# sefffal/Octofitter.jl

Hardware: AMD Instinct MI355X
Metric: epoch-likelihood evals/sec (fwd+grad), 1e4 epochs x 1e4 walkers (higher is better)
Workload: dtype f64; 1 GPU; config3: 1 planet, 10000 RA/Dec epochs x 10000 walkers in total (10000 walkers split over 1 GPUs: 10000 walkers/GPU), fwd+reverse-grad, inputs and outputs resident in HBM (PCIe-inclusive rate: value_pcie_inclusive); walkers_per_gpu=10000, walkers_total=10000, rows=10000, parallelism=walkers sharded x1, dataset replicated, no data-path collective

## Files before the change

### octofitter.jl_amd/csrc/octo_api.hip

```cpp
#define OCTO_API_TU 1
#include "octo_host.h"
#include "octo_tile.h"

using namespace octo;

namespace octo {

std::atomic<uint64_t> g_dataset_serial{1};

int fail(octo_ctx* ctx, int code, const std::string& msg) {
    if (ctx) ctx->err = msg;
    return code;
}

int busy(octo_ctx* ctx, const char* what) {
    if (ctx->pending.active) return fail(ctx, OCTO_EINVAL, std::string(what) + ": an octo_eval_begin of this context has not been ended");
    return OCTO_OK;
}


DevConsts dev_consts(const octo_consts& c) {
    DevConsts d;
    d.k_yr = c.kepler_year_to_julian_day; d.yd = c.year2day_julian; d.au2m = c.au2m; d.sec2yr = c.sec2year_julian;
    d.mas_per_au_per_plx = c.rad2as / c.pc2au;
// ... 219 lines not shown
    if (rounds != 1 || ctx->env_rounds > 0 || n_rows < 32 * WPB * 8) return key0;
    const int64_t t_max = std::max<int64_t>(1, n_rows / (32 * WPB));
    int64_t best_t = key0;
    double best_cost = 1e300;
    for (int wps = 1; wps <= blocks_per_cu; ++wps) {
        int64_t t = std::min<int64_t>((int64_t)wps * n_cus / cols, t_max);
        if (t < 1) continue;
        const double chunk = std::ceil((double)n_rows / (double)(t * WPB));
        const double n = std::ceil((double)(cols * t) / (double)n_cus);
        static const double g[8] = {1.59, 1.59, 1.13, 1.045, 1.03, 1.015, 1.005, 1.0};
        const double cost = n * g[(int)std::min(n, 7.0)] * (chunk + 2.7) + 0.34 * (double)t;
        if (cost < best_cost) { best_cost = cost; best_t = t; }
    }
    if (wide && ctx->env_wide >= 0) {
        const double n4 = std::ceil((double)(cols * best_t) / (double)n_cus);
        *wide = (n4 <= (double)blocks8_per_cu && n_rows >= (int64_t)best_t * 8 * 32) || (ctx->env_wide > 0 && n4 <= (double)blocks8_per_cu);
    }
    return best_t;
}

bool small_eligible(const octo_ctx* ctx, const octo_dataset* ds, int64_t W, bool model) {
    if (ctx->opt_invariant) return false;
    if (ds->n_planets > MAXP_T) return false;
    const int limit = (model && ds->n_planets == 1) ? std::max(ctx->small_w, ctx->small_w_model) : ctx->small_w;
    if (!(W * ds->n_planets <= limit && W <= SMALL_W)) return false;
    if (ds->kind_mask & KM_MARG)
        for (int o = 0; o < ds->n_obs; ++o)
            if (ds->h_obs[o].kind == OCTO_RV_ABS_MARG && ds->h_obs[o].n > SMALL_MARG_ROWS) return false;
    return true;
}

constexpr int TILE_PROBE_EVERY = 64;
constexpr double TILE_COLD_ROW_US = 27.0 * 2.15e-3;
constexpr double TILE_LAUNCH_US = 6.5;

static int tile_settle(octo_ctx* ctx, const octo_dataset* ds) {
    HIPCHK(ctx, hipEventSynchronize(ctx->ev_tile));
    double d = 0.0;
    for (int k = 0; k < ctx->tile_pending_segs; ++k) d += (double)ctx->h_tile_stats[2 * k] - (double)ctx->h_tile_stats[2 * k + 1];
    ctx->tile_last_saving_us = d * (double)ds->tile_rows * TILE_COLD_ROW_US / (4.0 * (double)ctx->n_cus);
    ctx->tile_on = ctx->tile_last_saving_us > 1.3 * TILE_LAUNCH_US;
    ctx->tile_pending = false;
    return OCTO_OK;
}

int tile_prepare(octo_ctx* ctx, const octo_dataset* ds, EvalArgs& a, hipStream_t st) {
    a.perm = nullptr;
    const int kp = ds->n_planets - 1;
    if (!a.warm || ctx->tile_mode == 0 || a.W < ctx->tile_min_w || !(ds->tile_dm_ref > 0.0f) || ds->n_planets > 2 ||
        ds->planets[kp].orbit_kind == OCTO_ORBIT_THIELE_INNES)
        return OCTO_OK;
    bool probe = false, sort_now = ctx->tile_mode == 1;
    if (ctx->tile_mode == 2 && ds->n_planets > 1) return OCTO_OK;
    if (ctx->tile_mode == 2) {
        if (ctx->tile_ds != ds->serial || ctx->tile_W != a.W) {
            ctx->tile_ds = ds->serial; ctx->tile_W = a.W; ctx->tile_seq = 0; ctx->tile_on = false; ctx->tile_pending = false;
        }
        if (ctx->tile_pending) { int rcd = tile_settle(ctx, ds); if (rcd) return rcd; }
        probe = (ctx->tile_seq % TILE_PROBE_EVERY) == 0;
        ctx->tile_seq += 1;
        sort_now = ctx->tile_on;
    }
    if (!sort_now && !probe) return OCTO_OK;
    const int n_seg = (int)((a.W + TILE_SEG - 1) / TILE_SEG);
    int rc = grow(ctx, ctx->d_perm, ctx->cap_perm, a.W);
    if (rc) return rc;
    if (2 * (int64_t)n_seg > ctx->cap_tile_stats) {
        if (ctx->h_tile_stats) ctx->retired_host.push_back((void*)ctx->h_tile_stats);
        ctx->h_tile_stats = nullptr; ctx->cap_tile_stats = 0;
        const int64_t n = 2 * (int64_t)n_seg + 64;
        HIPCHK(ctx, hipHostMalloc((void**)&ctx->h_tile_stats, sizeof(float) * (size_t)n, hipHostMallocMapped | hipHostMallocPortable | hipHostMallocCoherent));
        ctx->cap_tile_stats = n;
    }
    if (!ctx->ev_tile) HIPCHK(ctx, hipEventCreateWithFlags(&ctx->ev_tile, hipEventDisableTiming));
    TileArgs ta;
    ta.elems = a.elems; ta.ld = a.ld; ta.W = a.W; ta.perm = ctx->d_perm; ta.stats = probe ? ctx->h_tile_stats : nullptr;
    ta.dm_ref = ds->tile_dm_ref; ta.inv_k_yr = (float)(1.0 / ctx->consts.kepler_year_to_julian_day);
    ta.planet = kp; ta.pad = 0;
    hipLaunchKernelGGL(k_tile_sort, dim3((unsigned)n_seg), dim3(TILE_TPB), 0, st, ta);
    if (probe) {
        HIPCHK(ctx, hipEventRecord(ctx->ev_tile, st));
        ctx->tile_pending = true; ctx->tile_pending_segs = n_seg; ctx->tile_probes += 1;
        if (ctx->tile_seq == 1) {
            int rcd = tile_settle(ctx, ds);
            if (rcd) return rcd;
            sort_now = ctx->tile_on;
        }
    }
    if (sort_now) { ctx->tile_sorted_launches += 1; a.perm = ctx->d_perm; }
    return OCTO_OK;
}

int drain_timing(octo_ctx* ctx) {
    for (size_t k = 0; k < ctx->ev_used; ++k) {
        float ms = 0.f;
        HIPCHK(ctx, hipEventSynchronize(ctx->ev_pool[k].second));
        HIPCHK(ctx, hipEventElapsedTime(&ms, ctx->ev_pool[k].first, ctx->ev_pool[k].second));
        ctx->t_ms += ms;
        ctx->t_n += 1;
        if (ctx->t_samples.size() < (1u << 20)) ctx->t_samples.push_back(ms);
    }
    ctx->ev_used = 0;
    return OCTO_OK;
}

}

extern "C" {

int32_t octo_consts_default(octo_consts* out) {
    if (!out) return OCTO_EINVAL;
    out->kepler_year_to_julian_day = 365.2568983840419;
    out->year2day_julian = 365.25;
    out->au2m = 1.495978707e11;
    out->sec2year_julian = 3.168808781402895e-8;
// ... 676 lines not shown
    if (sorted_launches) *sorted_launches = ctx->tile_sorted_launches;
    if (probes) *probes = ctx->tile_probes;
    if (on) *on = ctx->tile_on ? 1 : 0;
    if (last_saving_us) *last_saving_us = ctx->tile_last_saving_us;
    return OCTO_OK;
}

int32_t octo_debug_kepler_warm(octo_ctx* ctx, const double* MA, const double* dM, const double* e, int64_t n, double* sinE_out, double* cosE_out,
                               double* used_warm_out) {
    if (!ctx || !MA || !dM || !e || !sinE_out || !cosE_out || !used_warm_out || n < 0) return fail(ctx, OCTO_EINVAL, "octo_debug_kepler_warm: null argument");
    { int rcb = busy(ctx, "octo_debug_kepler_warm"); if (rcb) return rcb; }
    if (n == 0) return OCTO_OK;
    HIPCHK(ctx, hipSetDevice(ctx->device));
    int rc = grow(ctx, ctx->d_in, ctx->cap_in, 3 * n);
    if (rc) return rc;
    rc = grow(ctx, ctx->d_out, ctx->cap_out, 3 * n);
    if (rc) return rc;
    hipStream_t st;
    { int rcs = use_stream(ctx, OCTO_STREAM_CTX, &st); if (rcs) return rcs; }
    HIPCHK(ctx, hipMemcpyAsync(ctx->d_in, MA, sizeof(double) * n, hipMemcpyHostToDevice, st));
    HIPCHK(ctx, hipMemcpyAsync(ctx->d_in + n, dM, sizeof(double) * n, hipMemcpyHostToDevice, st));
    HIPCHK(ctx, hipMemcpyAsync(ctx->d_in + 2 * n, e, sizeof(double) * n, hipMemcpyHostToDevice, st));
    hipLaunchKernelGGL(k_kepler_warm, dim3((unsigned)((n + 255) / 256)), dim3(256), sizeof(double) * 2 * SCT_N, st, ctx->d_in, ctx->d_in + n, ctx->d_in + 2 * n, n,
                       ctx->d_out, ctx->d_out + n, ctx->d_out + 2 * n, ctx->d_sctab);
    HIPCHK(ctx, hipGetLastError());
    HIPCHK(ctx, hipMemcpyAsync(sinE_out, ctx->d_out, sizeof(double) * n, hipMemcpyDeviceToHost, st));
    HIPCHK(ctx, hipMemcpyAsync(cosE_out, ctx->d_out + n, sizeof(double) * n, hipMemcpyDeviceToHost, st));
    HIPCHK(ctx, hipMemcpyAsync(used_warm_out, ctx->d_out + 2 * n, sizeof(double) * n, hipMemcpyDeviceToHost, st));
    HIPCHK(ctx, hipStreamSynchronize(st));
    free_retired(ctx);
    return OCTO_OK;
}

int32_t octo_kepler_solve(octo_ctx* ctx, const double* MA, const double* e, int64_t n, double* E_out, double* sinE_out,
                          double* cosE_out) {
    return kepler_solve_host(ctx, MA, e, n, E_out, sinE_out, cosE_out, false);
}

int32_t octo_kepler_solve_table(octo_ctx* ctx, const double* MA, const double* e, int64_t n, double* E_out, double* sinE_out,
                                double* cosE_out) {
    return kepler_solve_host(ctx, MA, e, n, E_out, sinE_out, cosE_out, true);
}

int32_t octo_timing_enable(octo_ctx* ctx, int32_t on) {
    if (!ctx) return OCTO_EINVAL;
    ctx->timing_every = on > 0 ? on : 0;
    ctx->timing_whole = on < 0;
    ctx->timing_seq = 0;
    return OCTO_OK;
}

int32_t octo_timing_read(octo_ctx* ctx, double* avg_ms, int64_t* n_launches, int32_t reset) {
    if (!ctx) return OCTO_EINVAL;
    HIPCHK(ctx, hipSetDevice(ctx->device));
    int rc = drain_timing(ctx);
    if (rc) return rc;
    if (avg_ms) *avg_ms = ctx->t_n > 0 ? ctx->t_ms / (double)ctx->t_n : 0.0;
    if (n_launches) *n_launches = ctx->t_n;
    if (reset) { ctx->t_ms = 0.0; ctx->t_n = 0; ctx->t_samples.clear(); }
    return OCTO_OK;
}

int32_t octo_timing_stats(octo_ctx* ctx, double* median_ms, double* min_ms, double* max_ms, int64_t* n_launches) {
    if (!ctx) return OCTO_EINVAL;
    HIPCHK(ctx, hipSetDevice(ctx->device));
    int rc = drain_timing(ctx);
// ... 504 lines not shown
```

### octofitter.jl_amd/csrc/octo_device.h

```cpp
#pragma once
#include <hip/hip_runtime.h>
#include <stdint.h>

namespace octo {

constexpr int WAVE = 64;
constexpr double PI = 3.141592653589793238462643383279502884;
constexpr double TWO_PI = 6.283185307179586476925286766559005768;
constexpr double PI2 = PI * PI;
constexpr double LOG2PI = 1.8378770664093454835606594728112;
constexpr double MK_K0 = 3.0 * PI2 / (PI2 - 6.0);
constexpr double MK_K1N = 8.0 * PI / (5.0 * (PI2 - 6.0));

enum : int {
    WC_INVP = 0,
    WC_TP,
    WC_E,
    WC_BETA,
    WC_EOB,
    WC_CB, WC_CG, WC_CA, WC_CF,
    WC_K,
    WC_COSW, WC_SINW,
    WC_MU,
    WC_A,
// ... 235 lines not shown
    const double u = s.dt * pc.invP;
    const double frac = u - rint(u);
    const float E1f = markley_starter_f32(frac, pc);
    const double E1 = (double)E1f;
    double s1, c1;
    if constexpr (TAB) sincos_table(E1f, tab, s1, c1);
    else sincos_halfangle(E1, s1, c1);
    const double f0 = fma(-pc.e, s1, fma(-frac, TWO_PI, E1));
    kepler_correct<INV_NR>(s, pc, E1, s1, c1, f0);
    return s;
}

template <int INV_NR>
__device__ __forceinline__ KSol kepler_warm_step(double t, const PC& pc, KWarm& st, double dm) {
    static_assert(INV_NR >= 0, "the warm start needs 1/(1 − e cos E) of every row");
    KSol s;
    s.dt = t - pc.tp;
    const double dM = dm * pc.invP;
    const double x = dM * st.invD;
    const double z = x * st.invD;
    const double dE = fma(-((pc.he * st.sE) * z), x, x);
    const double u = dE * dE;
    const double sr = dE * fma(u, fma(u, fma(u, OCTO_KT[22], OCTO_KT[17]), OCTO_KT[18]), 1.0);
    const double cm1 = u * fma(u, fma(u, fma(u, OCTO_KT[23], OCTO_KT[19]), OCTO_KT[20]), -0.5);
    const double ds = fma(st.sE, cm1, st.cE * sr);
    const double s1 = st.sE + ds;
    const double c1 = fma(st.cE, cm1, fma(-st.sE, sr, st.cE));
    const double f0 = fma(-pc.e, ds, dE - dM);
    kepler_correct<INV_NR, true>(s, pc, 0.0, s1, c1, f0);
    st.sE = s.sE; st.cE = s.cE; st.invD = s.invD;
    return s;
}

#ifndef OCTO_WARM_TRI
#define OCTO_WARM_TRI 1
#endif
template <int INV_NR, bool TRI = (OCTO_WARM_TRI != 0)>
__device__ __forceinline__ KSol kepler_solve_warm(double t, const PC& pc, const SinCosTab& tab, KWarm& st, double thr, double dm, bool row_ok = true) {
    static_assert(INV_NR >= 0, "the warm start needs 1/(1 − e cos E) of every row");
    KSol s;
    s.dt = t - pc.tp;
    double E1 = 0.0, s1, c1, f0;
    const bool warm_row = row_ok && __builtin_amdgcn_ballot_w64(st.invD >= thr) == 0;
    if constexpr (TRI) {
    {
        const double dM = dm * pc.invP;
        const double x = dM * st.invD;
        const double z = x * st.invD;
        const double dE = fma(-((pc.he * st.sE) * z), x, x);
        const double u = dE * dE;
        const double sr = dE * fma(u, fma(u, fma(u, OCTO_KT[22], OCTO_KT[17]), OCTO_KT[18]), 1.0);
        const double cm1 = u * fma(u, fma(u, fma(u, OCTO_KT[23], OCTO_KT[19]), OCTO_KT[20]), -0.5);
        const double ds = fma(st.sE, cm1, st.cE * sr);
        s1 = st.sE + ds;
        c1 = fma(st.cE, cm1, fma(-st.sE, sr, st.cE));
        f0 = fma(-pc.e, ds, dE - dM);
        kepler_correct<INV_NR, true>(s, pc, E1, s1, c1, f0);
    }
#ifndef OCTO_WARM_NOREDO
    if (__builtin_expect(!warm_row, 0)) {
        const double uo = s.dt * pc.invP;
        const double frac = uo - rint(uo);
        const float E1f = markley_starter_f32(frac, pc);
        E1 = (double)E1f;
        sincos_table(E1f, tab, s1, c1);
        f0 = fma(-pc.e, s1, fma(-frac, TWO_PI, E1));
// ... 33 lines not shown
```

### octofitter.jl_amd/csrc/octo_host.h

```cpp
#pragma once
#include <hip/hip_runtime.h>

#include <algorithm>
#include <atomic>
#include <cmath>
#include <cstdio>
#include <cstdlib>
#include <cstring>
#include <map>
#include <mutex>
#include <new>
#include <string>
#include <vector>

#include "octo_kernels.h"
#include "octo_model.h"
#include "octo_hgca.h"
#include "octo_small.h"
#include "octofitter_hip.h"

namespace octo {

struct TaskTable {
    uint64_t ds_serial = 0;
// ... 55 lines not shown
    double* d_marg = nullptr;
    double* d_extra = nullptr;
    int64_t cap_extra = 0;
    double* d_sctab = nullptr;
    int32_t* d_counters = nullptr;
    uint64_t* h_flags = nullptr;
    uint64_t flag_seq = 0;
    bool flag_request = false, flag_armed = false;
    SmallInline inl = {};
    int64_t stage_ws_in = 0, stage_ws_out = 0;
    struct ModelTail { const double *Jc = nullptr, *gtp = nullptr, *glp = nullptr, *lpp = nullptr; const octo_source *esrc = nullptr, *nsrc = nullptr; double *lp = nullptr, *grad = nullptr; int64_t ld = 0, ldo = 0; int32_t D = 0, n_nu = 0; };
    bool mt_applied = false;
    struct Pending {
        bool active = false, staged = false, walker_major = false;
        int64_t W = 0, ld = 0, ldd = 0, ws_out = 0, o_ge = 0, o_gn = 0;
        int n_el_out = 0, n_nu_out = 0;
        double *ll = nullptr, *g_elems = nullptr, *g_nuis = nullptr;
    } pending;
    void* comm = nullptr;
    int comm_rank = 0, comm_world = 1;
    int small_w_model = 768;
    int small_w = OCTO_SMALL_BATCH_DEFAULT;
    int64_t env_small_blocks = 0, env_small_min_span = 0, env_stage_bytes = 0, env_chunk = 0, env_rounds = 0, env_rv_cost = 0, env_kind_all = 0, env_mainp_tpb = 0;
    int env_warm = 1;
    int opt_warm = 1;
    int opt_invariant = 0;
    int tile_mode = 2;
    int64_t tile_min_w = 2048;
    int32_t* d_perm = nullptr; int64_t cap_perm = 0;
    float* h_tile_stats = nullptr; int64_t cap_tile_stats = 0;
    hipEvent_t ev_tile = nullptr;
    bool tile_on = false, tile_pending = false;
    int tile_pending_segs = 0;
    int64_t tile_seq = 0, tile_W = 0, tile_sorted_launches = 0, tile_probes = 0;
    uint64_t tile_ds = 0;
    double tile_last_saving_us = 0.0;
    int env_no_fin_fused = 0;
    int env_wide = 0;
    int flag_w = 128;
    int mapped_w = 128;
    double *d_in = nullptr, *d_out = nullptr;
    int64_t cap_in = 0, cap_out = 0;
    double *h_in = nullptr, *h_out = nullptr;
    int64_t cap_hin = 0, cap_hout = 0;
    std::vector<void*> retired_host;
    std::vector<void*> retired;
    std::vector<octo::TaskTable> tables;
    std::map<uint32_t, int> occupancy;
    std::map<const void*, size_t> lds_raised;
    int timing_every = 0;
    bool timing_whole = false;
    int64_t timing_seq = 0;
    std::vector<std::pair<hipEvent_t, hipEvent_t>> ev_pool;
    size_t ev_used = 0;
    double t_ms = 0.0;
    int64_t t_n = 0;
    std::vector<float> t_samples;
};


namespace octo {

int fail(octo_ctx* ctx, int code, const std::string& msg);

#define HIPCHK(ctx, call)                                                                          \
    do {                                                                                           \
// ... 57 lines not shown
```

### octofitter.jl_amd/csrc/octo_kernels.h

```cpp
#pragma once
#include <type_traits>

#include "octo_device.h"
#include "octofitter_hip.h"

namespace octo {

constexpr int MAXP = OCTO_MAX_PLANETS;
constexpr int MAXP_T = OCTO_MAX_PLANETS_ALL_KINDS;
constexpr int ROW_STRIDE = 8;
constexpr int WPB = 4;
#ifndef OCTO_FIN_G
#define OCTO_FIN_G 16
#endif
#ifndef OCTO_FIN_UNROLL
#define OCTO_FIN_UNROLL 4
#endif
constexpr int FIN_G = OCTO_FIN_G;
constexpr int fin_nwr(int n_planets) { return n_planets == 2 ? 3 : (n_planets == 3 ? 2 : 1); }
#ifndef OCTO_FIN_CH
#define OCTO_FIN_CH 6
#endif
#ifndef OCTO_FIN_FAST
#define OCTO_FIN_FAST true
// ... 288 lines not shown
    const KSol s = kepler_solve<2, TAB>(MA[i], pc, tab);
    const bool ok = (e >= 0.0) && (e < 1.0) && isfinite(MA[i]);
    E[i] = ok ? s.E : NAN;
    if (sE) sE[i] = ok ? s.sE : NAN;
    if (cE) cE[i] = ok ? s.cE : NAN;
}

static __global__ __launch_bounds__(256) void k_kepler_warm(const double* __restrict__ MA, const double* __restrict__ dMa, const double* __restrict__ ecc,
                                                            int64_t n, double* sE, double* cE, double* used, const double* __restrict__ sctab) {
    extern __shared__ __attribute__((aligned(16))) double lds[];
    const SinCosTab tab = make_sincos_tab(reinterpret_cast<const double2*>(lds));
    {
        const double2* __restrict__ g = reinterpret_cast<const double2*>(sctab);
        double2* t = reinterpret_cast<double2*>(lds);
        for (int i = threadIdx.x; i < SCT_N; i += blockDim.x) t[i] = g[i];
        __syncthreads();
    }
    const int64_t i0 = (int64_t)blockIdx.x * blockDim.x + threadIdx.x;
    const int64_t i = i0 < n ? i0 : n - 1;
    PC pc = {};
    const double e = ecc[i];
    pc.invP = 1.0 / TWO_PI; pc.tp = 0.0; pc.e = e; pc.beta = sqrt(1.0 - e * e); pc.eob = e / pc.beta;
    set_starter(pc, (float)e, (float)(1.0 - e), (float)(MK_K1N / (1.0 + e)));
    const KSol s0 = kepler_solve<2, true>(MA[i], pc, tab);
    KWarm st{s0.sE, s0.cE, s0.invD};
    const float dmx = fabsf((float)dMa[i]);
    double thr = (double)__builtin_amdgcn_exp2f(0.2f * (__builtin_amdgcn_logf((float)WARM_TOL) - 3.0f * __builtin_amdgcn_logf(dmx)));
    if (thr < WARM_MIN_THR) thr = 0.0;
    const bool warm = __builtin_amdgcn_ballot_w64(st.invD >= thr) == 0;
    const KSol s = kepler_solve_warm<2>(MA[i] + dMa[i], pc, tab, st, thr, dMa[i] * TWO_PI);
    if (i0 < n) { sE[i] = s.sE; cE[i] = s.cE; used[i] = warm ? 1.0 : 0.0; }
}

#endif

template <int P>
struct AstromCoef {
    double f[P];
    double jit, j2, ps, na, sn, cn;
    bool seppa, oneil;
    int planet, has_cor;
};

template <int P, bool GRAD, bool NUIS, int KM>
__device__ __forceinline__ AstromCoef<P> astrom_coef_vals(double jit, double ps, double na, int ob_kind, int ob_planet, int ob_has_cor, const PC (&pc)[P]) {
    using L = Layout<P, GRAD, NUIS, KM>;
    AstromCoef<P> c;
    if constexpr (P == 1) {
        c.f[0] = 1.0;
    } else {
        double a_this = 0.0;
#pragma unroll
        for (int p = 0; p < P; ++p) a_this = (p == ob_planet) ? pc[p].a : a_this;
#pragma unroll
        for (int p = 0; p < P; ++p) c.f[p] = (p == ob_planet) ? 1.0 : ((pc[p].a < a_this) ? pc[p].mu : 0.0);
    }
    c.jit = 0.0; c.j2 = 0.0; c.ps = 1.0; c.na = 0.0; c.sn = 0.0; c.cn = 1.0;
    if constexpr (NUIS) {
        c.jit = jit; c.ps = ps; c.na = na;
        sincos_reduced(c.na, c.sn, c.cn);
        c.j2 = c.jit * c.jit;
    }
    c.seppa = (KM & KM_SEPPA) && (ob_kind == OCTO_ASTROM_SEPPA || ob_kind == OCTO_ONEIL_SEPPA);
    c.oneil = L::HAS_ONEIL && (ob_kind == OCTO_ONEIL_RADEC || ob_kind == OCTO_ONEIL_SEPPA);
    c.planet = ob_planet; c.has_cor = ob_has_cor;
    return c;
}

template <int P, bool GRAD, bool NUIS, int KM>
__device__ __forceinline__ AstromCoef<P> astrom_coef(const double* __restrict__ nuis, int64_t ld, int ob_kind, int ob_planet, int ob_has_cor,
                                                     int obs_index, const PC (&pc)[P], int64_t wl) {
    double jit = 0.0, ps = 1.0, na = 0.0;
    if constexpr (NUIS) {
        const double* nu = nuis + (int64_t)obs_index * OCTO_N_NUIS * ld + wl;
        jit = nu[OCTO_NU_JITTER * ld]; ps = nu[OCTO_NU_PLATESCALE * ld]; na = nu[OCTO_NU_NORTHANGLE * ld];
    }
    return astrom_coef_vals<P, GRAD, NUIS, KM>(jit, ps, na, ob_kind, ob_planet, ob_has_cor, pc);
}

template <int P>
struct WarmState { KWarm st[P]; double thr[P]; uint32_t key_hi; bool row_ok; };

template <int P, bool GRAD, bool NUIS, int KM, bool TAB, int WARM = 0, bool WCHECK = true, int WLAST = 0>
__device__ __forceinline__ void astrom_row(AccArr<P, GRAD, NUIS, KM>& acc, LogProd& lp, const PC (&pc)[P],
                                           const AstromCoef<P>& co, double t, double y1, double y2, double c3, double c4, double c5,
                                           const SinCosTab& tab, WarmState<P>* ws = nullptr, double dm = 0.0) {
    using L = Layout<P, GRAD, NUIS, KM>;
    constexpr bool DEFER = TAB;
    const double (&f)[P] = co.f;
    const double jit = co.jit, j2 = co.j2, ps = co.ps, na = co.na, sn = co.sn, cn = co.cn;
    const bool seppa = co.seppa, oneil = co.oneil;
    KSol s[P];
    double rap[P], dep[P];
    double ra_m, dec_m;
#pragma unroll
    for (int p = 0; p < P; ++p) {
        if constexpr (WARM != 0) s[p] = kepler_solve_warm<1, WARM == 1>(t, pc[p], tab, ws->st[p], ws->thr[p], dm, WCHECK ? ws->row_ok : true);
        else if constexpr (WLAST != 0) { if (p == P - 1) s[p] = kepler_warm_step<1>(t, pc[p], ws->st[p], dm); else s[p] = kepler_solve<1, TAB>(t, pc[p], tab); }
        else s[p] = kepler_solve<1, TAB>(t, pc[p], tab);
        if constexpr (WLAST == 2) {
            if (p == P - 1 && __builtin_expect(!ws->row_ok, 0)) {
                s[p] = kepler_solve<1, TAB>(t, pc[p], tab);
                ws->st[p].sE = s[p].sE; ws->st[p].cE = s[p].cE; ws->st[p].invD = s[p].invD;
            }
        }
        rap[p] = fma(pc[p].cB, s[p].cE, fma(pc[p].cGb, s[p].sE, -pc[p].cBe));
        dep[p] = fma(pc[p].cA, s[p].cE, fma(pc[p].cFb, s[p].sE, -pc[p].cAe));
    }
    if constexpr (L::HAS_ONEIL) {
        if (oneil) {
            double sE = 0.0, cE = 0.0, ee = 0.0, invD = 0.0, dtp = 0.0;
#pragma unroll
            for (int p = 0; p < P; ++p) {
                const bool me = (P == 1) || (p == co.planet);
                sE = me ? s[p].sE : sE; cE = me ? s[p].cE : cE; ee = me ? pc[p].e : ee; invD = me ? s[p].invD : invD; dtp = me ? s[p].dt : dtp;
            }
            double E = 0.0;
#pragma unroll
            for (int p = 0; p < P; ++p) E = ((P == 1) || (p == co.planet)) ? s[p].E : E;
            const double Mm = fma(-ee, sE, E);
            const double c2 = fma(ee, ee + cE, -2.0);
            const double tt = fma(3.0 * Mm, ee + cE, 2.0 * c2 * sE);
            acc[L::OFF_ONEIL] += fabs(tt);
            if constexpr (GRAD) {
                const double sg = tt < 0.0 ? -1.0 : 1.0;
                const double D = fma(-ee, cE, 1.0);
                const double tM = 3.0 * (ee + cE);
                const double tE = fma(-3.0 * Mm, sE, 2.0 * fma(c2, cE, -(ee * sE * sE))) + tM * D;
                const double te = fma(2.0 * sE, 2.0 * ee + cE, 3.0 * Mm) - tM * sE;
                const double Mb = sg * tE * invD;
// ... 327 lines not shown
template <int P, bool GRAD, bool NUIS, int KM>
constexpr size_t main_lds_bytes() { return sizeof(double) * (2 * SCT_N + Layout<P, GRAD, NUIS, KM>::NACC * WAVE); }
template <int P, bool GRAD, bool NUIS, int KM, int NWV = WPB>
constexpr size_t fused_lds_bytes() {
    const size_t b = main_lds_bytes<P, GRAD, NUIS, KM>(), c = sizeof(double) * (size_t)P * NPC * WAVE;
    const size_t d = NWV > WPB ? sizeof(double) * (size_t)(NWV - 1) * Layout<P, GRAD, NUIS, KM>::NACC * WAVE : 0;
    return b > c ? (b > d ? b : d) : (c > d ? c : d);
}

template <int P, bool GRAD, bool NUIS, int KM, int NWV = WPB>
constexpr unsigned main_min_waves() {
    if (P >= 4 && GRAD) return 2u;
    if (NWV == 2 * WPB && P == 1 && GRAD && !NUIS && (KM & ~KM_COR) == KM_RADEC) return 6u;
#ifdef OCTO_P2_WAVES
    if (P == 2 && GRAD && NUIS && !(KM & (KM_MARG | KM_ONEIL))) return (unsigned)OCTO_P2_WAVES;
#endif
    return 1u;
}

#ifndef OCTO_WARM
#define OCTO_WARM 1
#endif
#ifndef OCTO_WARM_PLAIN
#define OCTO_WARM_PLAIN 0
#endif
template <int P, bool GRAD, bool NUIS, int KM, bool FUSED>
constexpr bool main_warm_plain() {
    return OCTO_WARM && FUSED && P == 1 && !(KM & KM_ONEIL) && NUIS && ((KM & KM_SEPPA) || ((KM & KM_RV) && OCTO_WARM_PLAIN));
}
template <int P, bool GRAD, bool NUIS, int KM, bool FUSED>
constexpr bool main_warm() {
    return OCTO_WARM && FUSED && P == 1 && !(KM & KM_ONEIL);
}

#ifndef OCTO_WARM_LAST3
#define OCTO_WARM_LAST3 1
#endif
template <int P, bool GRAD, bool NUIS, int KM, bool FUSED>
constexpr bool main_warm_last() {
    return OCTO_WARM && FUSED && (P == 2 || (P == 3 && OCTO_WARM_LAST3 && !(KM & KM_SEPPA))) && !(KM & (KM_ONEIL | KM_MARG));
}

template <int P>
__device__ __forceinline__ float warm_last_init(WarmState<P>& ws, const PC& pc, const DevObs& ob, bool enabled) {
    float bound = 0.0f;
#pragma unroll
    for (int k = WARM_LADDER - 1; k >= 0; --k) {
        const float d = enabled ? ob.dm_ladder[k] : 0.0f;
        const bool veto = fabsf(d * (float)pc.invP) > WARM_DM_VETO;
        if (d > 0.0f && __builtin_amdgcn_ballot_w64(veto) == 0) bound = d;
    }
    ws.key_hi = (uint32_t)__builtin_amdgcn_readfirstlane(__double2hiint((double)bound));
    const float dmx = fabsf(bound * (1.0f + 0x1p-18f) * (float)pc.invP);
    const float th = __builtin_amdgcn_exp2f(0.2f * (__builtin_amdgcn_logf((float)WARM_TOL) - 3.0f * __builtin_amdgcn_logf(dmx)));
    ws.thr[P - 1] = (double)th;
    ws.st[P - 1].sE = 0.0; ws.st[P - 1].cE = 1.0; ws.st[P - 1].invD = __builtin_huge_val();
    return bound;
}

template <int P>
__device__ __forceinline__ float warm_init(WarmState<P>& ws, const PC (&pc)[P], const DevObs& ob, bool enabled) {
    float bound = 0.0f;
#pragma unroll
    for (int k = WARM_LADDER - 1; k >= 0; --k) {
        const float d = enabled ? ob.dm_ladder[k] : 0.0f;
        bool veto = false;
// ... 101 lines not shown
            double v[NWC];
            setup_assemble(v, elv[p], a.orbit_kind[p], raw[0 * WAVE], raw[1 * WAVE], raw[2 * WAVE], raw[3 * WAVE], raw[4 * WAVE], raw[5 * WAVE], q);
            pc[p].invP = v[WC_INVP]; pc[p].tp = v[WC_TP]; pc[p].e = v[WC_E]; pc[p].beta = v[WC_BETA]; pc[p].eob = v[WC_EOB];
            pc[p].cB = v[WC_CB]; pc[p].cG = v[WC_CG]; pc[p].cA = v[WC_CA]; pc[p].cF = v[WC_CF]; pc[p].K = v[WC_K]; pc[p].cw = v[WC_COSW];
            pc[p].sw = v[WC_SINW]; pc[p].mu = v[WC_MU]; pc[p].a = v[WC_A]; pc[p].cGb = v[WC_CGB]; pc[p].cFb = v[WC_CFB]; pc[p].cBe = v[WC_CBE];
            pc[p].cAe = v[WC_CAE];
            const float2 fa = *reinterpret_cast<const float2*>(&v[WC_F32A]);
            const float2 fb = *reinterpret_cast<const float2*>(&v[WC_F32B]);
            set_starter(pc[p], fa.x, fa.y, fb.x);
        }
        __syncthreads();
        {
            double2* t = reinterpret_cast<double2*>(lds);
#pragma unroll
            for (int k = 0; k < TPT; ++k) { const int i = (int)threadIdx.x + k * WAVE * NWV; if (i < SCT_N) t[i] = make_double2(trs[k], trc[k]); }
        }
    }

    double acc[L::NACC];
#pragma unroll
    for (int k = 0; k < L::NACC; ++k) acc[k] = 0.0;
    LogProd lp;
    __syncthreads();

    const bool is_astrom = ob.kind == OCTO_ASTROM_RADEC || ob.kind == OCTO_ASTROM_SEPPA || ob.kind == OCTO_ONEIL_RADEC ||
                           ob.kind == OCTO_ONEIL_SEPPA;

    if (L::HAS_ASTROM && (!L::HAS_RV || is_astrom)) {
        const AstromCoef<P> co = astrom_coef<P, GRAD, NUIS, KM>(a.nuis, a.ld, ob.kind, ob.planet, ob.has_cor, tk.obs, pc, wsrc);
        const crow_t rows = constant_rows((NUIS ? ob.raw : ob.pre) + (int64_t)row_first * ROW_STRIDE);
        auto body = [&](const RowRegs& r) {
            astrom_row<P, GRAD, NUIS, KM, true>(acc, lp, pc, co, row_get(r, 0), row_get(r, 1), row_get(r, 2), row_get(r, 3), row_get(r, 4), row_get(r, 5), tab);
        };
        bool warm_loop = false, warm_unchecked = false;
        WarmState<P> ws;
        if constexpr (main_warm<P, GRAD, NUIS, KM, FUSED>()) {
            const float bound = warm_init<P>(ws, pc, ob, a.warm != 0);
            warm_loop = bound > 0.0f;
            warm_unchecked = warm_loop && tk.key_max <= bound && tk.chunk <= WARM_RESTART;
        }
        bool warm_last = false;
        if constexpr (main_warm_last<P, GRAD, NUIS, KM, FUSED>()) {
            const float bound = warm_last_init<P>(ws, pc[P - 1], ob, a.warm != 0);
            warm_last = bound > 0.0f && n_rows > 0;
        }
        if (main_warm_last<P, GRAD, NUIS, KM, FUSED>() && warm_last) {
            if constexpr (main_warm_last<P, GRAD, NUIS, KM, FUSED>()) {
                auto lbody = [&](const RowRegs8& r) {
                    const uint64_t over = __builtin_amdgcn_ballot_w64(ws.st[P - 1].invD >= ws.thr[P - 1]);
                    ws.row_ok = ((uint32_t)warm_row_ok<P>(ws, r) & (uint32_t)(over == 0)) != 0;
                    astrom_row<P, GRAD, NUIS, KM, true, 0, true, 2>(acc, lp, pc, co, row_get(r, 0), row_get(r, 1), row_get(r, 2), row_get(r, 3), row_get(r, 4),
                                                                        row_get(r, 5), tab, &ws, row_get(r, 6));
                };
                RowRegs8 A = row_issue8(rows);
                for (int j = 0; j < n_rows; j += 2) {
                    RowRegs8 B = row_wait_issue(A, rows + (int64_t)(j + 1 < n_rows ? j + 1 : j) * ROW_STRIDE);
                    lbody(A);
                    if (__builtin_expect(j + 1 >= n_rows, 0)) { row_drain(B); break; }
                    A = row_wait_issue(B, rows + (int64_t)(j + 2 < n_rows ? j + 2 : j + 1) * ROW_STRIDE);
                    lbody(B);
                }
                row_drain(A);
            }
        } else if constexpr (!ROW_PREFETCH) {
            for (int j = 0; j < n_rows; ++j) {
                const crow_t rw = rows + (int64_t)j * ROW_STRIDE;
                astrom_row<P, GRAD, NUIS, KM, true>(acc, lp, pc, co, rw[0], rw[1], rw[2], rw[3], rw[4], rw[5], tab);
            }
        } else if (main_warm<P, GRAD, NUIS, KM, FUSED>() && warm_loop) {
            if constexpr (main_warm_plain<P, GRAD, NUIS, KM, FUSED>()) {
                for (int j = 0; j < n_rows; ++j) {
                    const crow_t rw = rows + (int64_t)j * ROW_STRIDE;
                    ws.row_ok = (uint32_t)__double2hiint(rw[7]) <= ws.key_hi;
                    astrom_row<P, GRAD, NUIS, KM, true, WMODE, true>(acc, lp, pc, co, rw[0], rw[1], rw[2], rw[3], rw[4], rw[5], tab, &ws, rw[6]);
                }
            } else if constexpr (main_warm<P, GRAD, NUIS, KM, FUSED>()) {
                auto wbody_t = [&](const RowRegs8& r, auto checked) {
                    if constexpr (decltype(checked)::value) ws.row_ok = warm_row_ok<P>(ws, r);
                    astrom_row<P, GRAD, NUIS, KM, true, WMODE, decltype(checked)::value>(acc, lp, pc, co, row_get(r, 0), row_get(r, 1), row_get(r, 2), row_get(r, 3),
                                                                                         row_get(r, 4), row_get(r, 5), tab, &ws, row_get(r, 6));
                };
                auto wloop = [&](auto checked) {
                    RowRegs8 A = row_issue8(rows);
                    for (int j = 0; j < n_rows; j += 2) {
                        RowRegs8 B = row_wait_issue(A, rows + (int64_t)(j + 1 < n_rows ? j + 1 : j) * ROW_STRIDE);
                        wbody_t(A, checked);
                        if (__builtin_expect(j + 1 >= n_rows, 0)) { row_drain(B); break; }
                        A = row_wait_issue(B, rows + (int64_t)(j + 2 < n_rows ? j + 2 : j + 1) * ROW_STRIDE);
                        wbody_t(B, checked);
                    }
                    row_drain(A);
                };
                if (n_rows > 0) {
                    if (warm_unchecked) wloop(std::false_type{});
                    else wloop(std::true_type{});
                }
            }
        } else if (n_rows > 0) {
            RowRegs A = row_issue(rows);
            for (int j = 0; j < n_rows; j += 2) {
                RowRegs B = row_wait_issue(A, rows + (int64_t)(j + 1 < n_rows ? j + 1 : j) * ROW_STRIDE);
                body(A);
                if (__builtin_expect(j + 1 >= n_rows, 0)) { row_drain(B); break; }
                A = row_wait_issue(B, rows + (int64_t)(j + 2 < n_rows ? j + 2 : j + 1) * ROW_STRIDE);
                body(B);
            }
            row_drain(A);
        }
        astrom_finish_sums<P, GRAD, NUIS, KM>(acc, co);
    }
    if (L::HAS_RV && !is_astrom) {
        const RvCoef<P> co = rv_coef<P, GRAD, NUIS, KM>(a.nuis, a.ld, a.marg, a.ldw, ob.kind, ob.planet, tk.obs, pc, wsrc);
        const crow_t rows = constant_rows((NUIS ? ob.raw : ob.pre) + (int64_t)row_first * ROW_STRIDE);
        auto body = [&](const RowRegs& r) {
            rv_row<P, GRAD, NUIS, KM, true>(acc, lp, pc, co, row_get(r, 0), row_get(r, 1), row_get(r, 2), NUIS ? row_get(r, 3) : 0.0, tab);
        };
        bool warm_loop = false, warm_unchecked = false;
        WarmState<P> ws;
        if constexpr (main_warm<P, GRAD, NUIS, KM, FUSED>()) {
            const float bound = warm_init<P>(ws, pc, ob, a.warm != 0);
            warm_loop = bound > 0.0f;
            warm_unchecked = warm_loop && tk.key_max <= bound && tk.chunk <= WARM_RESTART;
        }
        bool warm_last = false;
        if constexpr (main_warm_last<P, GRAD, NUIS, KM, FUSED>()) {
            const float bound = warm_last_init<P>(ws, pc[P - 1], ob, a.warm != 0);
            warm_last = bound > 0.0f && n_rows > 0;
// ... 857 lines not shown
```

### octofitter.jl_amd/csrc/octo_tile.h

```cpp
#pragma once
#include "octo_kernels.h"

namespace octo {

#ifndef OCTO_TILE_WPT
#define OCTO_TILE_WPT 1
#endif
constexpr int TILE_WPT = OCTO_TILE_WPT;
constexpr int TILE_TPB = 1024;
constexpr int TILE_SEG = TILE_TPB * TILE_WPT;
constexpr int TILE_K = 32;

struct TileArgs {
    const double* elems;
    int64_t ld, W;
    int32_t* perm;
    float* stats;
    float dm_ref;
    float inv_k_yr;
    int32_t planet;
    int32_t pad;
};

__device__ __forceinline__ float wave_excl_scan(float x, int lane, float& total) {
    float s = x;
#pragma unroll
    for (int d = 1; d < WAVE; d <<= 1) {
        const float y = __shfl_up(s, d, WAVE);
        if (lane >= d) s += y;
    }
    total = __shfl(s, WAVE - 1, WAVE);
    return s - x;
}

#ifdef OCTO_API_TU
static __global__ __launch_bounds__(TILE_TPB) void k_tile_sort(TileArgs a) {
    __shared__ __attribute__((aligned(16))) uint8_t cnt[TILE_K * TILE_TPB];
    __shared__ uint16_t goff[TILE_K * WAVE];
    __shared__ uint16_t bbase[TILE_K + 1];
    __shared__ float slq[TILE_SEG];
    __shared__ float red[2 * (TILE_TPB / WAVE)];
    const int t = threadIdx.x, lane = t & (WAVE - 1), wv = t >> 6;
    const int64_t seg0 = (int64_t)blockIdx.x * TILE_SEG;
    const int n_seg = (int)(a.W - seg0 < TILE_SEG ? a.W - seg0 : TILE_SEG);
    {
        uint4* z = reinterpret_cast<uint4*>(cnt);
        z[t] = make_uint4(0, 0, 0, 0); z[t + TILE_TPB] = make_uint4(0, 0, 0, 0);
#pragma unroll
        for (int i = 0; i < TILE_WPT; ++i) slq[TILE_WPT * t + i] = 0.0f;
    }
    int bk[TILE_WPT]; float lq[TILE_WPT];
#pragma unroll
    for (int i = 0; i < TILE_WPT; ++i) {
        const int k = TILE_WPT * t + i;
        bk[i] = -1; lq[i] = 0.0f;
        if (k >= n_seg) continue;
        const int64_t w = seg0 + k;
        const double* el = a.elems + (int64_t)a.planet * OCTO_N_EL * a.ld + w;
        const double sma = el[(int64_t)OCTO_EL_A * a.ld], ecc = el[(int64_t)OCTO_EL_E * a.ld], Mt = el[(int64_t)OCTO_EL_M * a.ld];
        const float e = (float)ecc, af = (float)sma, mf = (float)Mt;
        const float invP = __builtin_amdgcn_rsqf(af * af * af * __builtin_amdgcn_rcpf(mf)) * a.inv_k_yr;
        const float dM = fabsf(a.dm_ref * invP);
        int b; float p;
        if (!(dM <= WARM_DM_VETO) || !(e >= 0.0f) || !(e < 1.0f)) {
            const float x = __builtin_amdgcn_logf(dM * (1.0f / WARM_DM_VETO)) * 2.0f;
            b = 25 + (x >= 0.0f ? (x < 6.0f ? (int)x : 6) : (x < 0.0f ? 0 : 6));
            p = 1.0f;
        } else {
            const float thr = __builtin_amdgcn_exp2f(0.2f * (__builtin_amdgcn_logf((float)WARM_TOL) - 3.0f * __builtin_amdgcn_logf(dM)));
            const float g = 1.0f - __builtin_amdgcn_rcpf(thr);
            if (e <= g) { b = 0; p = 0.0f; }
            else {
                const float c = g * __builtin_amdgcn_rcpf(e);
                const float E0 = __builtin_amdgcn_sqrtf(1.0f - c) * fmaf(fmaf(fmaf(-0.0187293f, c, 0.0742610f), c, -0.2121144f), c, 1.5707288f);
                const float s0 = __builtin_amdgcn_sqrtf(fmaxf(fmaf(-c, c, 1.0f), 0.0f));
                p = fminf(fmaxf((E0 - e * s0) * 0.318309886f, 0.0f), 1.0f);
                const float x = (__builtin_amdgcn_logf(fmaxf(p, 1e-30f)) + 17.0f) * (24.0f / 17.0f);
                b = 1 + (x > 0.0f ? (x < 23.0f ? (int)x : 23) : 0);
            }
        }
        bk[i] = b;
        lq[i] = p < 1.0f ? __builtin_amdgcn_logf(1.0f - p) : -INFINITY;
    }
    __syncthreads();
#pragma unroll
    for (int i = 0; i < TILE_WPT; ++i)
        if (bk[i] >= 0) cnt[bk[i] * TILE_TPB + t] += 1;
    __syncthreads();
#pragma unroll
    for (int q = 0; q < TILE_K / (TILE_TPB / WAVE); ++q) {
        const int b = wv * (TILE_K / (TILE_TPB / WAVE)) + q;
        uint4* grp = reinterpret_cast<uint4*>(cnt + b * TILE_TPB) + lane;
        uint4 v = *grp;
        uint32_t words[4] = {v.x, v.y, v.z, v.w};
        uint32_t run = 0;
#pragma unroll
        for (int wd = 0; wd < 4; ++wd) {
            uint32_t outw = 0;
#pragma unroll
            for (int by = 0; by < 4; ++by) {
                const uint32_t c = (words[wd] >> (8 * by)) & 0xffu;
                outw |= run << (8 * by);
                run += c;
            }
            words[wd] = outw;
        }
        *grp = make_uint4(words[0], words[1], words[2], words[3]);
        float tot;
        const float off = wave_excl_scan((float)run, lane, tot);
        goff[b * WAVE + lane] = (uint16_t)off;
        if (lane == 0) bbase[b + 1] = (uint16_t)tot;
    }
    __syncthreads();
    if (wv == 0) {
        static_assert(TILE_K <= WAVE, "one lane per bucket");
        const float c = lane < TILE_K ? (float)bbase[lane + 1] : 0.0f;
        float tot;
        const float off = wave_excl_scan(c, lane, tot);
        if (lane < TILE_K) bbase[lane] = (uint16_t)off;
    }
    __syncthreads();
#pragma unroll
    for (int i = 0; i < TILE_WPT; ++i) {
        if (bk[i] < 0) continue;
        int rank = 0;
#pragma unroll
        for (int j = 0; j < i; ++j) rank += (bk[j] == bk[i]) ? 1 : 0;
        const int pos = (int)bbase[bk[i]] + (int)goff[bk[i] * WAVE + (t >> 4)] + (int)cnt[bk[i] * TILE_TPB + t] + rank;
        a.perm[seg0 + pos] = (int32_t)(seg0 + TILE_WPT * t + i);
        slq[pos] = lq[i];
    }
    if (!a.stats) return;
    __syncthreads();
    constexpr int LPT = WAVE / TILE_WPT;
    float s_id = 0.0f, s_so = 0.0f;
#pragma unroll
    for (int i = 0; i < TILE_WPT; ++i) { s_id += lq[i]; s_so += slq[TILE_WPT * t + i]; }
#pragma unroll
    for (int d = 1; d < LPT; d <<= 1) { s_id += __shfl_xor(s_id, d, WAVE); s_so += __shfl_xor(s_so, d, WAVE); }
    const bool head = (lane & (LPT - 1)) == 0 && TILE_WPT * t < n_seg;
    float c_id = head ? 1.0f - __builtin_amdgcn_exp2f(s_id) : 0.0f;
    float c_so = head ? 1.0f - __builtin_amdgcn_exp2f(s_so) : 0.0f;
#pragma unroll
    for (int d = LPT; d < WAVE; d <<= 1) { c_id += __shfl_xor(c_id, d, WAVE); c_so += __shfl_xor(c_so, d, WAVE); }
    if (lane == 0) { red[2 * wv] = c_id; red[2 * wv + 1] = c_so; }
    __syncthreads();
    if (t == 0) {
        float x = 0.0f, y = 0.0f;
        for (int k = 0; k < TILE_TPB / WAVE; ++k) { x += red[2 * k]; y += red[2 * k + 1]; }
        a.stats[2 * blockIdx.x] = x; a.stats[2 * blockIdx.x + 1] = y;
    }
}
#endif

}
```

Before: 368.7 billion evals/s.

## Add fine warm-start Kepler step for tiny per-epoch anomaly increments

Adds a cheaper warm-start Kepler update that uses a truncated series rotation plus one Newton correction, with no checked fallback. It applies when every lane in a wavefront has a mean-anomaly step small relative to (1-e), in RA/Dec-only fused single-planet kernels. The tile sorter now puts fine-eligible walkers in a separate bucket, and the host cost model credits the expected savings when deciding whether to sort. The aim is to cut per-row Kepler solve cost. The risks are accuracy if the threshold is too loose, more code paths and register pressure, and a slightly different sorting heuristic.

```diff
diff --git a/octofitter.jl_amd/csrc/octo_api.hip b/octofitter.jl_amd/csrc/octo_api.hip
--- a/octofitter.jl_amd/csrc/octo_api.hip
+++ b/octofitter.jl_amd/csrc/octo_api.hip
@@ -275,13 +275,17 @@
 
 constexpr int TILE_PROBE_EVERY = 64;
 constexpr double TILE_COLD_ROW_US = 27.0 * 2.15e-3;
+constexpr double TILE_FINE_ROW_US = 20.0 * 2.15e-3;
 constexpr double TILE_LAUNCH_US = 6.5;
 
 static int tile_settle(octo_ctx* ctx, const octo_dataset* ds) {
     HIPCHK(ctx, hipEventSynchronize(ctx->ev_tile));
     double d = 0.0;
-    for (int k = 0; k < ctx->tile_pending_segs; ++k) d += (double)ctx->h_tile_stats[2 * k] - (double)ctx->h_tile_stats[2 * k + 1];
-    ctx->tile_last_saving_us = d * (double)ds->tile_rows * TILE_COLD_ROW_US / (4.0 * (double)ctx->n_cus);
+    for (int k = 0; k < ctx->tile_pending_segs; ++k) {
+        const float* sg = ctx->h_tile_stats + 4 * k;
+        d += ((double)sg[0] - (double)sg[1]) * TILE_COLD_ROW_US + (ctx->tile_fine ? ((double)sg[3] - (double)sg[2]) * TILE_FINE_ROW_US : 0.0);
+    }
+    ctx->tile_last_saving_us = d * (double)ds->tile_rows / (4.0 * (double)ctx->n_cus);
     ctx->tile_on = ctx->tile_last_saving_us > 1.3 * TILE_LAUNCH_US;
     ctx->tile_pending = false;
     return OCTO_OK;
@@ -308,10 +312,10 @@
     const int n_seg = (int)((a.W + TILE_SEG - 1) / TILE_SEG);
     int rc = grow(ctx, ctx->d_perm, ctx->cap_perm, a.W);
     if (rc) return rc;
-    if (2 * (int64_t)n_seg > ctx->cap_tile_stats) {
+    if (4 * (int64_t)n_seg > ctx->cap_tile_stats) {
         if (ctx->h_tile_stats) ctx->retired_host.push_back((void*)ctx->h_tile_stats);
         ctx->h_tile_stats = nullptr; ctx->cap_tile_stats = 0;
-        const int64_t n = 2 * (int64_t)n_seg + 64;
+        const int64_t n = 4 * (int64_t)n_seg + 64;
         HIPCHK(ctx, hipHostMalloc((void**)&ctx->h_tile_stats, sizeof(float) * (size_t)n, hipHostMallocMapped | hipHostMallocPortable | hipHostMallocCoherent));
         ctx->cap_tile_stats = n;
     }
@@ -324,6 +328,7 @@
     if (probe) {
         HIPCHK(ctx, hipEventRecord(ctx->ev_tile, st));
         ctx->tile_pending = true; ctx->tile_pending_segs = n_seg; ctx->tile_probes += 1;
+        ctx->tile_fine = a.nuis == nullptr && (ds->kind_mask & ~KM_COR) == KM_RADEC;
         if (ctx->tile_seq == 1) {
             int rcd = tile_settle(ctx, ds);
             if (rcd) return rcd;
@@ -1066,6 +1071,32 @@
     return OCTO_OK;
 }
 
+int32_t octo_debug_kepler_warm_fine(octo_ctx* ctx, const double* MA, const double* dM, const double* e, int64_t n, double* sinE_out, double* cosE_out,
+                               double* used_warm_out) {
+    if (!ctx || !MA || !dM || !e || !sinE_out || !cosE_out || !used_warm_out || n < 0) return fail(ctx, OCTO_EINVAL, "octo_debug_kepler_warm_fine: null argument");
+    { int rcb = busy(ctx, "octo_debug_kepler_warm_fine"); if (rcb) return rcb; }
+    if (n == 0) return OCTO_OK;
+    HIPCHK(ctx, hipSetDevice(ctx->device));
+    int rc = grow(ctx, ctx->d_in, ctx->cap_in, 3 * n);
+    if (rc) return rc;
+    rc = grow(ctx, ctx->d_out, ctx->cap_out, 3 * n);
+    if (rc) return rc;
+    hipStream_t st;
+    { int rcs = use_stream(ctx, OCTO_STREAM_CTX, &st); if (rcs) return rcs; }
+    HIPCHK(ctx, hipMemcpyAsync(ctx->d_in, MA, sizeof(double) * n, hipMemcpyHostToDevice, st));
+    HIPCHK(ctx, hipMemcpyAsync(ctx->d_in + n, dM, sizeof(double) * n, hipMemcpyHostToDevice, st));
+    HIPCHK(ctx, hipMemcpyAsync(ctx->d_in + 2 * n, e, sizeof(double) * n, hipMemcpyHostToDevice, st));
+    hipLaunchKernelGGL(k_kepler_warm_fine, dim3((unsigned)((n + 255) / 256)), dim3(256), sizeof(double) * 2 * SCT_N, st, ctx->d_in, ctx->d_in + n, ctx->d_in + 2 * n, n,
+                       ctx->d_out, ctx->d_out + n, ctx->d_out + 2 * n, ctx->d_sctab);
+    HIPCHK(ctx, hipGetLastError());
+    HIPCHK(ctx, hipMemcpyAsync(sinE_out, ctx->d_out, sizeof(double) * n, hipMemcpyDeviceToHost, st));
+    HIPCHK(ctx, hipMemcpyAsync(cosE_out, ctx->d_out + n, sizeof(double) * n, hipMemcpyDeviceToHost, st));
+    HIPCHK(ctx, hipMemcpyAsync(used_warm_out, ctx->d_out + 2 * n, sizeof(double) * n, hipMemcpyDeviceToHost, st));
+    HIPCHK(ctx, hipStreamSynchronize(st));
+    free_retired(ctx);
+    return OCTO_OK;
+}
+
 int32_t octo_kepler_solve(octo_ctx* ctx, const double* MA, const double* e, int64_t n, double* E_out, double* sinE_out,
                           double* cosE_out) {
     return kepler_solve_host(ctx, MA, e, n, E_out, sinE_out, cosE_out, false);
diff --git a/octofitter.jl_amd/csrc/octo_device.h b/octofitter.jl_amd/csrc/octo_device.h
--- a/octofitter.jl_amd/csrc/octo_device.h
+++ b/octofitter.jl_amd/csrc/octo_device.h
@@ -291,6 +291,33 @@
     return s;
 }
 
+constexpr float WARM_FINE_Q = 1.0e-3f;
+template <int INV_NR>
+__device__ __forceinline__ KSol kepler_warm_step_fine(double t, const PC& pc, KWarm& st, double dm) {
+    static_assert(INV_NR >= 0, "the warm start needs 1/(1 − e cos E) of every row");
+    KSol s;
+    s.dt = t - pc.tp;
+    const double dM = dm * pc.invP;
+    const double x = dM * st.invD;
+    const double z = x * st.invD;
+    const double dE = fma(-((pc.he * st.sE) * z), x, x);
+    const double u = dE * dE;
+    const double sr = dE * fma(u, OCTO_KT[18], 1.0);
+    const double cm1 = u * fma(u, OCTO_KT[20], -0.5);
+    const double ds = fma(st.sE, cm1, st.cE * sr);
+    const double s1 = st.sE + ds;
+    const double c1 = fma(st.cE, cm1, fma(-st.sE, sr, st.cE));
+    const double f0 = fma(-pc.e, ds, dE - dM);
+    const double r1 = rcp_nr<1>(fma(-pc.e, c1, 1.0));
+    const double d = -f0 * r1;
+    s.E = d;
+    s.sE = fma(c1, d, s1);
+    s.cE = fma(-s1, d, c1);
+    s.invD = fma(fma(-fma(-pc.e, s.cE, 1.0), r1, 1.0), r1, r1);
+    st.sE = s.sE; st.cE = s.cE; st.invD = s.invD;
+    return s;
+}
+
 #ifndef OCTO_WARM_TRI
 #define OCTO_WARM_TRI 1
 #endif
diff --git a/octofitter.jl_amd/csrc/octo_host.h b/octofitter.jl_amd/csrc/octo_host.h
--- a/octofitter.jl_amd/csrc/octo_host.h
+++ b/octofitter.jl_amd/csrc/octo_host.h
@@ -111,6 +111,7 @@
     hipEvent_t ev_tile = nullptr;
     bool tile_on = false, tile_pending = false;
     int tile_pending_segs = 0;
+    bool tile_fine = false;
     int64_t tile_seq = 0, tile_W = 0, tile_sorted_launches = 0, tile_probes = 0;
     uint64_t tile_ds = 0;
     double tile_last_saving_us = 0.0;
diff --git a/octofitter.jl_amd/csrc/octo_kernels.h b/octofitter.jl_amd/csrc/octo_kernels.h
--- a/octofitter.jl_amd/csrc/octo_kernels.h
+++ b/octofitter.jl_amd/csrc/octo_kernels.h
@@ -344,6 +344,29 @@
     if (i0 < n) { sE[i] = s.sE; cE[i] = s.cE; used[i] = warm ? 1.0 : 0.0; }
 }
 
+static __global__ __launch_bounds__(256) void k_kepler_warm_fine(const double* __restrict__ MA, const double* __restrict__ dMa, const double* __restrict__ ecc,
+                                                                 int64_t n, double* sE, double* cE, double* used, const double* __restrict__ sctab) {
+    extern __shared__ __attribute__((aligned(16))) double lds[];
+    const SinCosTab tab = make_sincos_tab(reinterpret_cast<const double2*>(lds));
+    {
+        const double2* __restrict__ g = reinterpret_cast<const double2*>(sctab);
+        double2* t = reinterpret_cast<double2*>(lds);
+        for (int i = threadIdx.x; i < SCT_N; i += blockDim.x) t[i] = g[i];
+        __syncthreads();
+    }
+    const int64_t i0 = (int64_t)blockIdx.x * blockDim.x + threadIdx.x;
+    const int64_t i = i0 < n ? i0 : n - 1;
+    PC pc = {};
+    const double e = ecc[i];
+    pc.invP = 1.0 / TWO_PI; pc.tp = 0.0; pc.e = e; pc.beta = sqrt(1.0 - e * e); pc.eob = e / pc.beta;
+    set_starter(pc, (float)e, (float)(1.0 - e), (float)(MK_K1N / (1.0 + e)));
+    const KSol s0 = kepler_solve<1, true>(MA[i], pc, tab);
+    KWarm st{s0.sE, s0.cE, s0.invD};
+    const bool fine = !(fabsf((float)dMa[i]) > WARM_FINE_Q * pc.omef);
+    const KSol s = kepler_warm_step_fine<1>(MA[i] + dMa[i], pc, st, dMa[i] * TWO_PI);
+    if (i0 < n) { sE[i] = s.sE; cE[i] = s.cE; used[i] = fine ? 1.0 : 0.0; }
+}
+
 #endif
 
 template <int P>
@@ -407,7 +430,8 @@
     double ra_m, dec_m;
 #pragma unroll
     for (int p = 0; p < P; ++p) {
-        if constexpr (WARM != 0) s[p] = kepler_solve_warm<1, WARM == 1>(t, pc[p], tab, ws->st[p], ws->thr[p], dm, WCHECK ? ws->row_ok : true);
+        if constexpr (WARM == 3) s[p] = kepler_warm_step_fine<1>(t, pc[p], ws->st[p], dm);
+        else if constexpr (WARM != 0) s[p] = kepler_solve_warm<1, WARM == 1>(t, pc[p], tab, ws->st[p], ws->thr[p], dm, WCHECK ? ws->row_ok : true);
         else if constexpr (WLAST != 0) { if (p == P - 1) s[p] = kepler_warm_step<1>(t, pc[p], ws->st[p], dm); else s[p] = kepler_solve<1, TAB>(t, pc[p], tab); }
         else s[p] = kepler_solve<1, TAB>(t, pc[p], tab);
         if constexpr (WLAST == 2) {
@@ -801,6 +825,10 @@
 constexpr bool main_warm() {
     return OCTO_WARM && FUSED && P == 1 && !(KM & KM_ONEIL);
 }
+template <int P, bool GRAD, bool NUIS, int KM, bool FUSED, int NWV>
+constexpr bool main_warm_fine() {
+    return main_warm<P, GRAD, NUIS, KM, FUSED>() && NWV == WPB && !NUIS && (KM & ~KM_COR) == KM_RADEC;
+}
 
 #ifndef OCTO_WARM_LAST3
 #define OCTO_WARM_LAST3 1
@@ -968,12 +996,14 @@
         auto body = [&](const RowRegs& r) {
             astrom_row<P, GRAD, NUIS, KM, true>(acc, lp, pc, co, row_get(r, 0), row_get(r, 1), row_get(r, 2), row_get(r, 3), row_get(r, 4), row_get(r, 5), tab);
         };
-        bool warm_loop = false, warm_unchecked = false;
+        bool warm_loop = false, warm_unchecked = false, warm_fine = false;
         WarmState<P> ws;
         if constexpr (main_warm<P, GRAD, NUIS, KM, FUSED>()) {
             const float bound = warm_init<P>(ws, pc, ob, a.warm != 0);
             warm_loop = bound > 0.0f;
             warm_unchecked = warm_loop && tk.key_max <= bound && tk.chunk <= WARM_RESTART;
+            if (main_warm_fine<P, GRAD, NUIS, KM, FUSED, NWV>() && warm_unchecked)
+                warm_fine = __builtin_amdgcn_ballot_w64(fabsf(bound * (1.0f + 0x1p-18f) * (float)pc[0].invP) > WARM_FINE_Q * pc[0].omef) == 0;
         }
         bool warm_last = false;
         if constexpr (main_warm_last<P, GRAD, NUIS, KM, FUSED>()) {
@@ -1027,8 +1057,30 @@
                     }
                     row_drain(A);
                 };
+                auto fbody = [&](const RowRegs8& r, double dm) {
+                    astrom_row<P, GRAD, NUIS, KM, true, 3, false>(acc, lp, pc, co, row_get(r, 0), row_get(r, 1), row_get(r, 2), row_get(r, 3), row_get(r, 4),
+                                                                  row_get(r, 5), tab, &ws, dm);
+                };
+                auto floop = [&]() {
+                  if constexpr (main_warm_fine<P, GRAD, NUIS, KM, FUSED, NWV>()) {
+                    RowRegs8 A = row_issue8(rows);
+                    for (int j = 0; j < n_rows; j += 2) {
+                        RowRegs8 B = row_wait_issue(A, rows + (int64_t)(j + 1 < n_rows ? j + 1 : j) * ROW_STRIDE);
+                        if (__builtin_expect(j == 0, 0)) {
+                            const KSol s0 = kepler_solve<1, true>(row_get(A, 0), pc[0], tab);
+                            ws.st[0].sE = s0.sE; ws.st[0].cE = s0.cE; ws.st[0].invD = s0.invD;
+                        }
+                        fbody(A, j == 0 ? 0.0 : row_get(A, 6));
+                        if (__builtin_expect(j + 1 >= n_rows, 0)) { row_drain(B); break; }
+                        A = row_wait_issue(B, rows + (int64_t)(j + 2 < n_rows ? j + 2 : j + 1) * ROW_STRIDE);
+                        fbody(B, row_get(B, 6));
+                    }
+                    row_drain(A);
+                  }
+                };
                 if (n_rows > 0) {
-                    if (warm_unchecked) wloop(std::false_type{});
+                    if (warm_fine) floop();
+                    else if (warm_unchecked) wloop(std::false_type{});
                     else wloop(std::true_type{});
                 }
             }
diff --git a/octofitter.jl_amd/csrc/octo_tile.h b/octofitter.jl_amd/csrc/octo_tile.h
--- a/octofitter.jl_amd/csrc/octo_tile.h
+++ b/octofitter.jl_amd/csrc/octo_tile.h
@@ -39,7 +39,7 @@
     __shared__ uint16_t goff[TILE_K * WAVE];
     __shared__ uint16_t bbase[TILE_K + 1];
     __shared__ float slq[TILE_SEG];
-    __shared__ float red[2 * (TILE_TPB / WAVE)];
+    __shared__ float red[3 * (TILE_TPB / WAVE)];
     const int t = threadIdx.x, lane = t & (WAVE - 1), wv = t >> 6;
     const int64_t seg0 = (int64_t)blockIdx.x * TILE_SEG;
     const int n_seg = (int)(a.W - seg0 < TILE_SEG ? a.W - seg0 : TILE_SEG);
@@ -50,6 +50,7 @@
         for (int i = 0; i < TILE_WPT; ++i) slq[TILE_WPT * t + i] = 0.0f;
     }
     int bk[TILE_WPT]; float lq[TILE_WPT];
+    bool nf = false;
 #pragma unroll
     for (int i = 0; i < TILE_WPT; ++i) {
         const int k = TILE_WPT * t + i;
@@ -66,17 +67,20 @@
             const float x = __builtin_amdgcn_logf(dM * (1.0f / WARM_DM_VETO)) * 2.0f;
             b = 25 + (x >= 0.0f ? (x < 6.0f ? (int)x : 6) : (x < 0.0f ? 0 : 6));
             p = 1.0f;
+            nf = true;
         } else {
             const float thr = __builtin_amdgcn_exp2f(0.2f * (__builtin_amdgcn_logf((float)WARM_TOL) - 3.0f * __builtin_amdgcn_logf(dM)));
             const float g = 1.0f - __builtin_amdgcn_rcpf(thr);
-            if (e <= g) { b = 0; p = 0.0f; }
+            const bool fine = !(dM * (1.0f + 0x1p-18f) > WARM_FINE_Q * (1.0f - e));
+            nf = nf || !fine;
+            if (fine || e <= g) { b = fine ? 0 : 1; p = 0.0f; }
             else {
                 const float c = g * __builtin_amdgcn_rcpf(e);
                 const float E0 = __builtin_amdgcn_sqrtf(1.0f - c) * fmaf(fmaf(fmaf(-0.0187293f, c, 0.0742610f), c, -0.2121144f), c, 1.5707288f);
                 const float s0 = __builtin_amdgcn_sqrtf(fmaxf(fmaf(-c, c, 1.0f), 0.0f));
                 p = fminf(fmaxf((E0 - e * s0) * 0.318309886f, 0.0f), 1.0f);
-                const float x = (__builtin_amdgcn_logf(fmaxf(p, 1e-30f)) + 17.0f) * (24.0f / 17.0f);
-                b = 1 + (x > 0.0f ? (x < 23.0f ? (int)x : 23) : 0);
+                const float x = (__builtin_amdgcn_logf(fmaxf(p, 1e-30f)) + 17.0f) * (23.0f / 17.0f);
+                b = 2 + (x > 0.0f ? (x < 22.0f ? (int)x : 22) : 0);
             }
         }
         bk[i] = b;
@@ -133,22 +137,24 @@
     if (!a.stats) return;
     __syncthreads();
     constexpr int LPT = WAVE / TILE_WPT;
-    float s_id = 0.0f, s_so = 0.0f;
+    float s_id = 0.0f, s_so = 0.0f, n_id = nf ? 1.0f : 0.0f;
 #pragma unroll
     for (int i = 0; i < TILE_WPT; ++i) { s_id += lq[i]; s_so += slq[TILE_WPT * t + i]; }
 #pragma unroll
-    for (int d = 1; d < LPT; d <<= 1) { s_id += __shfl_xor(s_id, d, WAVE); s_so += __shfl_xor(s_so, d, WAVE); }
+    for (int d = 1; d < LPT; d <<= 1) { s_id += __shfl_xor(s_id, d, WAVE); s_so += __shfl_xor(s_so, d, WAVE); n_id += __shfl_xor(n_id, d, WAVE); }
     const bool head = (lane & (LPT - 1)) == 0 && TILE_WPT * t < n_seg;
     float c_id = head ? 1.0f - __builtin_amdgcn_exp2f(s_id) : 0.0f;
     float c_so = head ? 1.0f - __builtin_amdgcn_exp2f(s_so) : 0.0f;
+    float f_id = (head && n_id == 0.0f) ? 1.0f : 0.0f;
 #pragma unroll
-    for (int d = LPT; d < WAVE; d <<= 1) { c_id += __shfl_xor(c_id, d, WAVE); c_so += __shfl_xor(c_so, d, WAVE); }
-    if (lane == 0) { red[2 * wv] = c_id; red[2 * wv + 1] = c_so; }
+    for (int d = LPT; d < WAVE; d <<= 1) { c_id += __shfl_xor(c_id, d, WAVE); c_so += __shfl_xor(c_so, d, WAVE); f_id += __shfl_xor(f_id, d, WAVE); }
+    if (lane == 0) { red[3 * wv] = c_id; red[3 * wv + 1] = c_so; red[3 * wv + 2] = f_id; }
     __syncthreads();
     if (t == 0) {
-        float x = 0.0f, y = 0.0f;
-        for (int k = 0; k < TILE_TPB / WAVE; ++k) { x += red[2 * k]; y += red[2 * k + 1]; }
-        a.stats[2 * blockIdx.x] = x; a.stats[2 * blockIdx.x + 1] = y;
+        float x = 0.0f, y = 0.0f, z = 0.0f;
+        for (int k = 0; k < TILE_TPB / WAVE; ++k) { x += red[3 * k]; y += red[3 * k + 1]; z += red[3 * k + 2]; }
+        a.stats[4 * blockIdx.x] = x; a.stats[4 * blockIdx.x + 1] = y;
+        a.stats[4 * blockIdx.x + 2] = z; a.stats[4 * blockIdx.x + 3] = (float)(bbase[1] / WAVE);
     }
 }
 #endif
```

Measured after the change: 380.0 billion evals/s, median of 6. 3.1% higher.
